# li-kunyi/CUT3R-SLAM

Hardware: AMD Instinct MI355X
Metric: frames/sec (ViT pointmap + covisibility-graph tracking step) on 640x480 (higher is better)
Workload: dtype f16

## Files before the change

cut3r_slam_amd/_lib.py:

```python
from __future__ import annotations

import ctypes as C
import os

_HERE = os.path.dirname(os.path.abspath(__file__))
LIB_PATH = os.path.join(_HERE, "libcut3r_hip.so")

c_void_p, c_int, c_float, c_ll = C.c_void_p, C.c_int, C.c_float, C.c_longlong


class GemmDesc(C.Structure):
    _fields_ = [
        ("A", c_void_p), ("B", c_void_p), ("C", c_void_p), ("bias", c_void_p), ("res1", c_void_p), ("res2", c_void_p),
        ("M", c_int), ("N", c_int), ("K", c_int), ("lda", c_int), ("ldb", c_int), ("ldc", c_int), ("ldr1", c_int),
        ("ldr2", c_int),
        ("act", c_int), ("out_f16", c_int), ("res1_f16", c_int), ("res2_f16", c_int),
        ("batch", c_int),
        ("strideA", c_ll), ("strideB", c_ll), ("strideC", c_ll), ("strideBias", c_ll), ("strideR1", c_ll),
        ("strideR2", c_ll),
        ("conv_k", c_int), ("H", c_int), ("W", c_int), ("Cin", c_int), ("conv_stride", c_int), ("Ho", c_int),
        ("Wo", c_int), ("relu_in", c_int),
        ("shuf", c_int), ("shuf_cout", c_int), ("shuf_Hin", c_int), ("shuf_Win", c_int),
        ("tile", c_int), ("stages", c_int),
        ("rope_pos", c_void_p), ("rope_table", c_void_p), ("rope_cols", c_int), ("rope_pmin", c_int), ("rope_npos", c_int),
# ... 13 lines not shown
    "cut3r_rope2d_qk": [c_void_p, c_void_p, c_int, c_void_p, c_int, c_int, c_int, c_int, c_ll, c_ll, c_ll, c_ll, c_float, c_float,
                        c_void_p],
    "cut3r_rope2d_tab": [c_void_p, c_void_p, c_ll, c_ll, c_void_p, c_void_p, c_ll, c_ll, c_int, c_int, c_void_p, c_int, c_int, c_float,
                         c_float, c_void_p],
    "cut3r_layernorm": [c_void_p, c_int, c_void_p, c_void_p, c_float, c_int, c_int, c_void_p, c_int, c_void_p, c_int,
                        c_void_p, c_void_p, c_void_p],
    "cut3r_layernorm_dual": [c_void_p, c_int, c_void_p, c_void_p, c_void_p, c_int, c_void_p, c_void_p, c_void_p, c_int, c_float, c_int,
                             c_int, c_void_p],
    "cut3r_gemm_f16": [C.POINTER(GemmDesc), c_void_p],
    "cut3r_gemm_tile_for": [C.POINTER(GemmDesc)],
    "cut3r_gemm_f16_pair": [C.POINTER(GemmDesc), C.POINTER(GemmDesc), c_void_p],
    "cut3r_rope2d_table": [c_void_p, c_int, c_int, c_int, c_float, c_float, c_void_p],
    "cut3r_gemv_f16w": [c_void_p, c_int, c_void_p, c_int, c_void_p, c_void_p, c_int, c_int, c_int, c_int, c_int,
                        c_void_p, c_int, c_int, c_void_p],
    "cut3r_attention_variant": [c_int],
    "cut3r_attention_f16": [c_void_p, c_void_p, c_void_p, c_void_p, c_int, c_int, c_int, c_int, c_int,
                            c_ll, c_ll, c_ll, c_ll, c_ll, c_ll, c_ll, c_ll, c_float, c_void_p],
    "cut3r_im2col_patch": [c_void_p, c_int, c_int, c_int, c_int, c_int, c_int, c_void_p, c_void_p],
    "cut3r_cast_f32_f16": [c_void_p, c_int, c_void_p, c_int, c_int, c_int, c_void_p],
    "cut3r_colmean": [c_void_p, c_int, c_int, c_int, c_void_p, c_void_p],
    "cut3r_colmean_batched": [c_void_p, c_int, c_ll, c_int, c_int, c_int, c_void_p, c_ll, c_void_p],
    "cut3r_upsample2x_nhwc": [c_void_p, c_void_p, c_int, c_int, c_int, c_int, c_void_p],
    "cut3r_dpt_final": [c_void_p, c_int, c_int, c_void_p, c_void_p, c_int, c_void_p, c_void_p, c_void_p],
    "cut3r_postprocess_pts": [c_void_p, c_int, c_int, c_int, c_void_p, c_void_p, c_void_p],
    "cut3r_postprocess_pose": [c_void_p, c_int, c_void_p, c_void_p],
    "cut3r_patch_overlap": [c_void_p, c_void_p, c_int, c_int, c_float, c_void_p, c_void_p, c_void_p],
    "cut3r_patch_overlap_chain": [c_void_p, c_void_p, c_int, c_int, c_int, c_float, C.c_double, c_void_p, c_void_p, c_void_p, c_void_p,
                                  c_void_p, c_void_p],
    "cut3r_overlap_fwd": [c_void_p, c_int, C.POINTER(c_float), c_float, c_void_p, c_int, c_float, c_float, c_float, c_float,
                          c_int, c_int, c_int, c_void_p, c_void_p],
# ... 119 lines not shown
```

cut3r_slam_amd/csrc/attention.hip:

```cpp
#include <atomic>
#include <cstdlib>
#include <type_traits>
#include "common.h"
#include "../../include/cut3r_hip.h"

namespace {

typedef __fp16 fp16x4_t __attribute__((ext_vector_type(4)));

DEVINL void halves(float x, float& lo, float& hi) {
    const auto r = __builtin_amdgcn_permlane32_swap(__float_as_uint(x), __float_as_uint(x), false, false);
    lo = __uint_as_float(r[0]);
    hi = __uint_as_float(r[1]);
}

struct AttnArgs {
    const h16* q; const h16* k; const h16* v; h16* o;
    int Nq, Nk;
    long long q_sb, q_sn, k_sb, k_sn, v_sb, v_sn, o_sb, o_sn;
    float scale_log2;
};

template <int D, int NW>
__global__ __launch_bounds__(NW * 64, (D <= 64 && NW == 4) ? 3 : 1) void attn_kernel(const AttnArgs a) {
    constexpr int NTHR = NW * 64;
    constexpr int KT = 64;
    constexpr int DQ = D / 16;
    constexpr int DP = (D + 31) / 32;
    constexpr int KS_LD = D + 8;
    constexpr int VS_BYTES = (64 * DP) % 128 == 0 ? 64 * DP + 64 : 64 * DP;
    constexpr int V_LD = VS_BYTES / 2;
    constexpr int CHUNKS = KT * (D / 8);
    constexpr int NCH = (CHUNKS + NTHR - 1) / NTHR;
    __shared__ __attribute__((aligned(16))) h16 Ks[KT * KS_LD];
    __shared__ __attribute__((aligned(16))) h16 Vs[KT * V_LD];

// ... 2 lines not shown
    const int h = blockIdx.y, b = blockIdx.z;
    const int q0 = blockIdx.x * (32 * NW) + wave * 32;
    const h16* qp = a.q + (size_t)b * a.q_sb + (size_t)h * D;
    const h16* kp = a.k + (size_t)b * a.k_sb + (size_t)h * D;
    const h16* vp = a.v + (size_t)b * a.v_sb + (size_t)h * D;

    for (int i = tid; i < KT * V_LD; i += NTHR) Vs[i] = (h16)0;

    half8_t qf[DQ];
    {
        int qr = q0 + r;
        if (qr > a.Nq - 1) qr = a.Nq - 1;
        const h16* qrow = qp + (size_t)qr * a.q_sn;
#pragma unroll
        for (int s = 0; s < DQ; s++) qf[s] = *reinterpret_cast<const half8_t*>(qrow + 16 * s + 8 * hh);
    }

    f32x16 ot[DP];
#pragma unroll
    for (int d = 0; d < DP; d++)
#pragma unroll
        for (int i = 0; i < 16; i++) ot[d][i] = 0.f;
    float m_run = -INFINITY, l_run = 0.f;
    const bool active = q0 < a.Nq;
    const int extra = (a.Nk > KT && (a.Nk % KT) == 1) ? 1 : 0;
    if (extra) {
        float dot = 0.f;
#pragma unroll
        for (int s = 0; s < DQ; s++) {
            const half8_t k0 = *reinterpret_cast<const half8_t*>(kp + 16 * s + 8 * hh);
// ... 265 lines not shown
        }
        asm volatile("s_waitcnt vmcnt(0)" ::: "memory");
        return;
    }

    half8_t qf[QB][DQ];
    f32x16 ot[QB][DP];
    float m_run[QB], l_run[QB];
#pragma unroll
    for (int qb = 0; qb < QB; qb++) {
        int qr = q0 + qb * 32 + r;
        if (qr > a.Nq - 1) qr = a.Nq - 1;
        const h16* qrow = qp + (size_t)qr * a.q_sn;
#pragma unroll
        for (int s = 0; s < DQ; s++) qf[qb][s] = *reinterpret_cast<const half8_t*>(qrow + 16 * s + 8 * hh);
#pragma unroll
        for (int d = 0; d < DP; d++)
#pragma unroll
            for (int i = 0; i < 16; i++) ot[qb][d][i] = 0.f;
        m_run[qb] = -INFINITY;
        l_run[qb] = 0.f;
        if (extra) {
            float dot = 0.f;
#pragma unroll
            for (int s = 0; s < DQ; s++) {
                const half8_t k0 = *reinterpret_cast<const half8_t*>(kp + 16 * s + 8 * hh);
#pragma unroll
                for (int j = 0; j < 8; j++) dot = fmaf((float)qf[qb][s][j], (float)k0[j], dot);
            }
            { float d0, d1; halves(dot, d0, d1); dot = d0 + d1; }
// ... 250 lines not shown
            dim3 grid((unsigned)(((HB + 7) / 8) * 8 * nblk));
            hipLaunchKernelGGL((attn_pipe_kernel<D, 1, 4, 4>), grid, dim3(256), 0, s, a, nblk, HB, H);
            return cut3r_check_launch();
        }
    }
    if (blocks128 >= nw4_min || D >= 128) {
        dim3 grid((a.Nq + 127) / 128, H, B);
        hipLaunchKernelGGL((attn_kernel<D, 4>), grid, dim3(256), 0, s, a);
    } else {
        dim3 grid((a.Nq + 63) / 64, H, B);
        hipLaunchKernelGGL((attn_kernel<D, 2>), grid, dim3(128), 0, s, a);
    }
    return cut3r_check_launch();
}

}

extern "C" int cut3r_attention_variant(int v) {
    if (v < 0) return g_attn_variant.load(std::memory_order_relaxed);
    return g_attn_variant.exchange(v ? 1 : 0, std::memory_order_relaxed);
}

extern "C" int cut3r_attention_f16(const void* q, const void* k, const void* v, void* out, int B, int H, int Nq, int Nk, int D,
                                   long long q_sb, long long q_sn, long long k_sb, long long k_sn, long long v_sb, long long v_sn,
                                   long long o_sb, long long o_sn, float scale, void* stream) {
    if (!q || !k || !v || !out || B <= 0 || H <= 0 || Nq <= 0 || Nk <= 0) return CUT3R_ERR_ARG;
    if (((uintptr_t)q | (uintptr_t)k | (uintptr_t)v) & 15) return CUT3R_ERR_ARG;
    if ((uintptr_t)out & 7) return CUT3R_ERR_ARG;
    if ((q_sn | k_sn | v_sn | q_sb | k_sb | v_sb) & 7) return CUT3R_ERR_ARG;
    if ((o_sn | o_sb) & 3) return CUT3R_ERR_ARG;
    AttnArgs a;
    a.q = (const h16*)q; a.k = (const h16*)k; a.v = (const h16*)v; a.o = (h16*)out;
    a.Nq = Nq; a.Nk = Nk;
    a.q_sb = q_sb; a.q_sn = q_sn; a.k_sb = k_sb; a.k_sn = k_sn; a.v_sb = v_sb; a.v_sn = v_sn; a.o_sb = o_sb; a.o_sn = o_sn;
    a.scale_log2 = scale * 1.44269504088896340736f;
    hipStream_t s = (hipStream_t)stream;
    switch (D) {
        case 16: return launch_attn<16>(a, B, H, s);
        case 32: return launch_attn<32>(a, B, H, s);
        case 48: return launch_attn<48>(a, B, H, s);
        case 64: return launch_attn<64>(a, B, H, s);
        case 128: return launch_attn<128>(a, B, H, s);
        default: return CUT3R_ERR_ARG;
    }
}
```

cut3r_slam_amd/csrc/elementwise.hip:

```cpp
#include "common.h"
#include "../../include/cut3r_hip.h"

namespace {

template <typename T> struct alignas(4 * sizeof(T)) Vec4 { T v[4]; };

template <typename T>
__global__ __launch_bounds__(256) void rope2d_kernel(T* __restrict__ tok, T* __restrict__ tok2, const int64_t* __restrict__ pos,
                                                     int N, int H, int D, long long sB, long long sN, long long sH, long long sB2,
                                                     long long sN2, float base, float fwd) {
    __shared__ float cs[2][2][64];
    const int t = blockIdx.x;
    const int b = t / N, n = t - b * N;
    const int Q = D >> 2;
    if (threadIdx.x < 2 * Q) {
        const int X = threadIdx.x / Q, q = threadIdx.x - X * Q;
        const float inv = fwd / powf(base, (float)q / (float)Q);
        const float fr = (float)pos[(size_t)t * 2 + X] * inv;
        cs[X][0][q] = cosf(fr);
        cs[X][1][q] = sinf(fr);
    }
    __syncthreads();
    const int Q4 = Q >> 2;
    const int per_tensor = H * 2 * Q4;
// ... 265 lines not shown
        *reinterpret_cast<half8_t*>(out + m * Kp + k) = o;
    }
}

__global__ __launch_bounds__(256) void cast_kernel(const float* __restrict__ x, int ldx, h16* __restrict__ y, int ldy, int M, int C4) {
    const size_t total = (size_t)M * C4;
    for (size_t i = blockIdx.x * (size_t)blockDim.x + threadIdx.x; i < total; i += (size_t)gridDim.x * blockDim.x) {
        const int c = (int)(i % C4);
        const size_t m = i / C4;
        f32x4 v = *reinterpret_cast<const f32x4*>(x + m * ldx + c * 4);
        half4_t o = {(h16)v[0], (h16)v[1], (h16)v[2], (h16)v[3]};
        *reinterpret_cast<half4_t*>(y + m * ldy + c * 4) = o;
    }
}

__global__ __launch_bounds__(256) void colmean_kernel(const float* __restrict__ x, int ldx, int M, int C, float* __restrict__ y,
                                                      long long sx, long long sy) {
    __shared__ float part[16][64];
    x += (size_t)blockIdx.y * sx;
    y += (size_t)blockIdx.y * sy;
    const int col = threadIdx.x & 63, rg = threadIdx.x >> 6;
    const int c = blockIdx.x * 64 + col;
    float s0 = 0.f, s1 = 0.f, s2 = 0.f, s3 = 0.f;
    if (c < C) {
        int m = rg;
        for (; m + 12 < M; m += 16) {
            s0 += x[(size_t)m * ldx + c];
            s1 += x[(size_t)(m + 4) * ldx + c];
            s2 += x[(size_t)(m + 8) * ldx + c];
            s3 += x[(size_t)(m + 12) * ldx + c];
// ... 319 lines not shown
    if (!img || !out || B <= 0 || C <= 0 || P <= 0 || (P & 7) || H % P || W % P) return CUT3R_ERR_ARG;
    const size_t total = (size_t)B * (H / P) * (W / P) * (C * P * P / 8);
    if (u8)
        hipLaunchKernelGGL((im2col_kernel<true>), dim3(grid_for(total)), dim3(256), 0, (hipStream_t)stream, img, B, C, H, W, P, (h16*)out);
    else
        hipLaunchKernelGGL((im2col_kernel<false>), dim3(grid_for(total)), dim3(256), 0, (hipStream_t)stream, img, B, C, H, W, P, (h16*)out);
    return cut3r_check_launch();
}

extern "C" int cut3r_cast_f32_f16(const float* x, int ldx, void* y, int ldy, int M, int C, void* stream) {
    if (!x || !y || M <= 0 || C <= 0 || (C & 3) || (ldx & 3) || (ldy & 3)) return CUT3R_ERR_ARG;
    hipLaunchKernelGGL(cast_kernel, dim3(grid_for((size_t)M * (C / 4))), dim3(256), 0, (hipStream_t)stream, x, ldx, (h16*)y, ldy, M, C / 4);
    return cut3r_check_launch();
}

extern "C" int cut3r_colmean(const float* x, int ldx, int M, int C, float* y, void* stream) {
    if (!x || !y || M <= 0 || C <= 0) return CUT3R_ERR_ARG;
    hipLaunchKernelGGL(colmean_kernel, dim3((C + 63) / 64), dim3(256), 0, (hipStream_t)stream, x, ldx, M, C, y, 0LL, 0LL);
    return cut3r_check_launch();
}

extern "C" int cut3r_colmean_batched(const float* x, int B, long long stride_x, int ldx, int M, int C, float* y, long long stride_y,
                                     void* stream) {
    if (!x || !y || B <= 0 || B > 65535 || M <= 0 || C <= 0) return CUT3R_ERR_ARG;
    hipLaunchKernelGGL(colmean_kernel, dim3((C + 63) / 64, B), dim3(256), 0, (hipStream_t)stream, x, ldx, M, C, y, stride_x, stride_y);
    return cut3r_check_launch();
}

extern "C" int cut3r_upsample2x_nhwc(const void* in, void* out, int B, int H, int W, int C, void* stream) {
    if (!in || !out || B <= 0 || H <= 0 || W <= 0 || C <= 0 || (C & 7)) return CUT3R_ERR_ARG;
// ... 51 lines not shown
```

cut3r_slam_amd/model.py:

```python
from __future__ import annotations

import gc

import math
import re
from dataclasses import dataclass
from typing import Dict, List, Optional

import torch

from . import ops
from .config import Cut3rConfig, production_config, state_dict_schema

F16, F32 = torch.float16, torch.float32


@dataclass
class ARCroco3DStereoOutput:
    ress: Optional[List[dict]] = None
    views: Optional[List[dict]] = None


class _Lin:

# ... 31 lines not shown
        self.dual_stream = _os.environ.get("CUT3R_DUAL_STREAM", "1") != "0"
        self.dual_ln = _os.environ.get("CUT3R_DUAL_LN", "1") != "0"
        self.pair_gemm = _os.environ.get("CUT3R_PAIR_GEMM", "0") != "0"
        self.pair_rows = int(_os.environ.get("CUT3R_PAIR_ROWS", "0"))
        self.fused_rope = int(_os.environ.get("CUT3R_FUSED_ROPE", "1"))
        self.rope48_rows = int(_os.environ.get("CUT3R_ROPE48_ROWS", "0"))
        self.head_overlap = _os.environ.get("CUT3R_HEAD_OVERLAP", "1") != "0"
        self.head_chunk = max(1, int(_os.environ.get("CUT3R_HEAD_CHUNK", "28")))
        self.ln_fold = int(_os.environ.get("CUT3R_LN_FOLD", "1"))
        self._head_stream = None
        self._side = None
        self._head_side = None
        self.kv_fork = _os.environ.get("CUT3R_KV_FORK", "0") != "0"
        self.kv_fork_rows = int(_os.environ.get("CUT3R_KV_FORK_ROWS", "2048"))
        self._kv_streams = None
        self._prep(state_dict)

    @classmethod
    def from_state_dict(cls, cfg, sd, device="cuda:0", **kw):
        return cls(cfg, sd, device, **kw)

    @classmethod
    def from_pretrained(cls, path: str, config: Optional[Cut3rConfig] = None, device="cuda:0", **kw):
        import argparse
        import os
        if not os.path.isfile(path):
            raise FileNotFoundError(f"{path}: no checkpoint (this runtime never fetches from a hub)")
        with torch.serialization.safe_globals([argparse.Namespace]):
            ckpt = torch.load(path, map_location="cpu", weights_only=True)
        sd = ckpt["model"] if "model" in ckpt else ckpt
# ... 24 lines not shown
            self.w[name] = _Lin(sd[key + ".weight"], sd.get(key + ".bias"), dev)

        def ln(name):
            self.w[name] = (f32(name + ".weight"), f32(name + ".bias"))

        def fold(name, w, b, norm):
            if not self.ln_fold or w.shape[1] % 64 or w.shape[0] % 4:
                return
            gam, bet = sd[norm + ".weight"].double(), sd[norm + ".bias"].double()
            wd = w.double()
            L = _Lin((wd * gam[None, :]).float(), None, dev)
            L.b = (wd @ bet + b.double()).to(device=dev, dtype=F32).contiguous()
            L.c = L.w.double().sum(1).to(F32).contiguous()
            self.w[name + "@ln"] = L

        def enc_block(p):
            ln(p + ".norm1"); lin(p + ".attn.qkv"); lin(p + ".attn.proj"); ln(p + ".norm2")
            lin(p + ".mlp.fc1"); lin(p + ".mlp.fc2")
            if self.ln_fold >= 2:
                fold(p + ".attn.qkv", sd[p + ".attn.qkv.weight"], sd[p + ".attn.qkv.bias"], p + ".norm1")
                fold(p + ".mlp.fc1", sd[p + ".mlp.fc1.weight"], sd[p + ".mlp.fc1.bias"], p + ".norm2")

        def dec_block(p, folded=True):
            ln(p + ".norm1"); lin(p + ".attn.qkv"); lin(p + ".attn.proj")
            ln(p + ".norm2"); ln(p + ".norm3"); ln(p + ".norm_y")
            lin(p + ".cross_attn.projq"); lin(p + ".cross_attn.proj")
            wkv = torch.cat([sd[p + ".cross_attn.projk.weight"], sd[p + ".cross_attn.projv.weight"]], 0)
            bkv = torch.cat([sd[p + ".cross_attn.projk.bias"], sd[p + ".cross_attn.projv.bias"]], 0)
            self.w[p + ".cross_attn.projkv"] = _Lin(wkv, bkv, dev)
            lin(p + ".mlp.fc1"); lin(p + ".mlp.fc2")
            if folded:
                fold(p + ".attn.qkv", sd[p + ".attn.qkv.weight"], sd[p + ".attn.qkv.bias"], p + ".norm1")
                fold(p + ".cross_attn.projq", sd[p + ".cross_attn.projq.weight"], sd[p + ".cross_attn.projq.bias"], p + ".norm2")
                fold(p + ".cross_attn.projkv", wkv, bkv, p + ".norm_y")
                fold(p + ".mlp.fc1", sd[p + ".mlp.fc1.weight"], sd[p + ".mlp.fc1.bias"], p + ".norm3")

        self.w["patch_embed"] = _Lin(sd["patch_embed.proj.weight"], sd["patch_embed.proj.bias"], dev)
        for i in range(cfg.enc_depth):
            enc_block(f"enc_blocks.{i}")
        ln("enc_norm")
        lin("decoder_embed"); lin("decoder_embed_state")
        for i in range(cfg.dec_depth):
            dec_block(f"dec_blocks.{i}"); dec_block(f"dec_blocks_state.{i}")
        ln("dec_norm"); ln("dec_norm_state")
        lin("pose_retriever.proj_q")
        for i in range(2):
            dec_block(f"pose_retriever.write_blocks.{i}", False); dec_block(f"pose_retriever.read_blocks.{i}", False)
# ... 86 lines not shown
        def prob(x, name, out, res, ex):
            ex = dict(ex or {})
            L = self.w[name + "@ln"] if ex.get("ln") is not None else self.w[name]
            if ex.get("ln") is not None:
                ex["ln"] = (ex["ln"], L.c, self.cfg.ln_eps)
            if ex.get("rope") is not None:
                r = ex["rope"]
                ex["rope"] = (r[0], r[1], self.cfg.rope_freq, r[2])
            return (x, L.w, out, L.b, res, {k: v for k, v in ex.items() if v is not None})
        ops.linear_pair(prob(x0, name0, out0, res0, ex0), prob(x1, name1, out1, res1, ex1), act)

    def _fuse_rope(self, pos, D, rows):
        dims = (64, 48) if (self.fused_rope == 2 or (self.fused_rope and rows <= self.rope48_rows)) else (64,)
        return self.fused_rope and pos is not None and D in dims and pos.is_contiguous() and pos.numel() == 2 * rows

    def _ln(self, x, name, out16=None, out32=None, mod=None):
        g, b = self.w[name]
        ops.layernorm(x, g, b, self.cfg.ln_eps, out16, out32, mod[0] if mod else None, mod[1] if mod else None)

    def _rope(self, t, pos):
        ops.rope_2d_pair(t, pos, None, None, self.cfg.rope_freq, 1.0)

    def _self_attn(self, tag, x_ln16, B, N, heads, pos, p, out, res, ln=None, emit=None):
        Cc = x_ln16.shape[1]
        D = Cc // heads
        sk = N == 1
        qkv = self.buf(tag + ".qkv", (B * N, 3 * Cc), F16)
        fuse = (not sk) and self._fuse_rope(pos, D, B * N)
        self._linear(x_ln16, p + ".qkv", qkv, skinny=sk, rope=(pos, 2 * Cc, D) if fuse else None, ln=ln)
        v5 = qkv.view(B, N, 3, heads, D)
        q, k, v = v5[:, :, 0], v5[:, :, 1], v5[:, :, 2]
        if pos is not None and not fuse:
            ops.rope_2d_pair(q, pos, k, pos, self.cfg.rope_freq, 1.0)
        a = self.buf(tag + ".attn", (B, N, heads, D), F16)
        ops.attention(q, k, v, a, D ** -0.5)
        self._linear(a.view(B * N, Cc), p + ".proj", out, res1=res, skinny=sk, emit=emit)

    def _mlp(self, tag, x_ln16, p, out, res, skinny=False, ln=None, emit=None):
        M = x_ln16.shape[0]
        hdim = self.w[p + ".fc1"].npad
        h = self.buf(tag + ".mlp_h", (M, hdim), F16)
        self._linear(x_ln16, p + ".fc1", h, act=1, skinny=skinny, ln=ln)
        self._linear(h, p + ".fc2", out, res1=res, skinny=skinny, emit=emit)

    def _encode(self, img: torch.Tensor):
        cfg = self.cfg
        B, _, H, W = img.shape
        P, E = cfg.patch_size, cfg.enc_embed_dim
        nh, nw = H // P, W // P
        N = nh * nw
# ... 98 lines not shown
                if not pre_ln:
                    self._ln(y, p + ".norm_y", out16=y16)
                self._linear(y16, p + ".cross_attn.projkv", kv, skinny=(Ny == 1), rope=(ypos, Cc, D) if fuse_k else None)
            if ypos is not None and not fuse_k:
                self._rope(k, ypos)

        if kv_only:
            kv_branch()
            return None
        if xs is not None:
            self._self_attn(tag, xs[0], B, Nx, heads, xpos, p + ".attn", out, x, ln=xs[1], emit=em)
        else:
            if not pre_ln:
                self._ln(x, p + ".norm1", out16=ln16)
            self._self_attn(tag, ln16, B, Nx, heads, xpos, p + ".attn", out, x, emit=em)
        q = self.buf(tag + ".q", (B, Nx, heads, D), F16)
        fuse_q = Nx > 1 and self._fuse_rope(xpos, D, B * Nx)
        if os_ is not None:
            self._linear(os_[0], p + ".cross_attn.projq", q.view(B * Nx, Cc), rope=(xpos, Cc, D) if fuse_q else None, ln=os_[1])
        else:
            self._ln(out, p + ".norm2", out16=ln16)
            self._linear(ln16, p + ".cross_attn.projq", q.view(B * Nx, Cc), skinny=(Nx == 1), rope=(xpos, Cc, D) if fuse_q else None)
        if xpos is not None and not fuse_q:
            self._rope(q, xpos)
        if kv_stream is not None:
            torch.cuda.current_stream().wait_stream(kv_stream)
        else:
            kv_branch()
        a = self.buf(tag + ".cattn", (B, Nx, heads, D), F16)
        ops.attention(q, k, v, a, D ** -0.5)
        self._linear(a.view(B * Nx, Cc), p + ".cross_attn.proj", out, res1=out, skinny=(Nx == 1), emit=em)
        if os_ is not None:
            self._mlp(tag, os_[0], p + ".mlp", out, out, ln=os_[1], emit=em)
        else:
            self._ln(out, p + ".norm3", out16=ln16)
            self._mlp(tag, ln16, p + ".mlp", out, out, skinny=(Nx == 1))
        return out

    def _dec_layer_pair(self, l, a, s_a, b, s_b, pos_img, pos_state, Wn, fork=False, xs=None, os_=None):
        cfg = self.cfg
        Cc = a.shape[1]
        ps, pi = f"dec_blocks_state.{l}", f"dec_blocks.{l}"
        Ni, Ns = a.shape[0] // Wn, s_a.shape[0] // Wn
        hs, hi = cfg.state_dec_num_heads, cfg.dec_num_heads
        Ds, Di = Cc // hs, Cc // hi
# ... 27 lines not shown
                    fn(S)
                fn(I)
                cur.wait_stream(self._side)
            else:
                fn(S)
                fn(I)

        if not fold_in:
            if self.dual_ln and Cc in (768, 1024, 1536):
                self._dual_norms(l, a, s_a)
            else:
                both(lambda sd: (self._ln(sd["x"], sd["p"] + ".norm1", out16=sd["ln16"]), self._ln(sd["y"], sd["p"] + ".norm_y", out16=sd["y16"])))
        for sd in (S, I):
            sd["fq"] = fr(sd["xpos"], sd["D"], Wn * sd["Nx"])
            sd["fk"] = fr(sd["ypos"], sd["D"], Wn * sd["Ny"])
        ex = lambda sd: {"rope": (sd["xpos"], 2 * Cc, sd["D"]) if sd["fq"] else None, "ln": sd["xst"] if fold_in else None}
        self._linear_pair(S["x16"] if fold_in else S["ln16"], ps + ".attn.qkv", S["qkv"], I["x16"] if fold_in else I["ln16"], pi + ".attn.qkv", I["qkv"],
                          ex0=ex(S), ex1=ex(I))

        def self_attn(sd):
            v5 = sd["qkv"].view(Wn, sd["Nx"], 3, sd["heads"], sd["D"])
            q, k, v = v5[:, :, 0], v5[:, :, 1], v5[:, :, 2]
            if sd["xpos"] is not None and not sd["fq"]:
                ops.rope_2d_pair(q, sd["xpos"], k, sd["xpos"], cfg.rope_freq, 1.0)
            ops.attention(q, k, v, sd["att"], sd["D"] ** -0.5)
        both(self_attn)
        self._linear_pair(S["att"].view(Wn * Ns, Cc), ps + ".attn.proj", S["out"], I["att"].view(Wn * Ni, Cc), pi + ".attn.proj", I["out"],
                          res0=S["x"], res1=I["x"], ex0=em(S), ex1=em(I))
        if not fold_out:
            both(lambda sd: self._ln(sd["out"], sd["p"] + ".norm2", out16=sd["ln16"]))
        ex = lambda sd: {"rope": (sd["xpos"], Cc, sd["D"]) if sd["fq"] else None, "ln": sd["ost"] if fold_out else None}
        self._linear_pair(S["o16"] if fold_out else S["ln16"], ps + ".cross_attn.projq", S["q"].view(Wn * Ns, Cc),
                          I["o16"] if fold_out else I["ln16"], pi + ".cross_attn.projq", I["q"].view(Wn * Ni, Cc), ex0=ex(S), ex1=ex(I))
        exk = lambda sd, other: {"rope": (sd["ypos"], Cc, sd["D"]) if sd["fk"] else None, "ln": other["xst"] if fold_in else None}
        self._linear_pair(I["x16"] if fold_in else S["y16"], ps + ".cross_attn.projkv", S["kv"], S["x16"] if fold_in else I["y16"], pi + ".cross_attn.projkv", I["kv"],
                          ex0=exk(S, I), ex1=exk(I, S))

        def cross_attn(sd):
            kv4 = sd["kv"].view(Wn, sd["Ny"], 2, sd["heads"], sd["D"])
            k, v = kv4[:, :, 0], kv4[:, :, 1]
            if not sd["fq"] or not sd["fk"]:
                qq = sd["q"] if not sd["fq"] else None
                kk = k if not sd["fk"] else None
                if qq is not None and kk is not None:
                    ops.rope_2d_pair(qq, sd["xpos"], kk, sd["ypos"], cfg.rope_freq, 1.0)
                elif qq is not None:
                    self._rope(qq, sd["xpos"])
                elif kk is not None:
                    self._rope(kk, sd["ypos"])
            ops.attention(sd["q"], k, v, sd["catt"], sd["D"] ** -0.5)
        both(cross_attn)
        self._linear_pair(S["catt"].view(Wn * Ns, Cc), ps + ".cross_attn.proj", S["out"], I["catt"].view(Wn * Ni, Cc), pi + ".cross_attn.proj", I["out"],
                          res0=S["out"], res1=I["out"], ex0=em(S), ex1=em(I))
        if not fold_out:
            both(lambda sd: self._ln(sd["out"], sd["p"] + ".norm3", out16=sd["ln16"]))
        ex = lambda sd: {"ln": sd["ost"] if fold_out else None}
        self._linear_pair(S["o16"] if fold_out else S["ln16"], ps + ".mlp.fc1", S["h"], I["o16"] if fold_out else I["ln16"], pi + ".mlp.fc1", I["h"], act=1,
                          ex0=ex(S), ex1=ex(I))
        self._linear_pair(S["h"], ps + ".mlp.fc2", S["out"], I["h"], pi + ".mlp.fc2", I["out"], res0=S["out"], res1=I["out"], ex0=em(S), ex1=em(I))

    def _dual_norms(self, l, a, s_a):
        pi, ps = f"dec_blocks.{l}", f"dec_blocks_state.{l}"
        Ci = a.shape[1]
        ops.layernorm_dual(a, *self.w[pi + ".norm1"], self.buf("deci.ln16", (a.shape[0], Ci), F16),
                           *self.w[ps + ".norm_y"], self.buf("decs.y16", (a.shape[0], Ci), F16), self.cfg.ln_eps)
# ... 421 lines not shown
```

cut3r_slam_amd/ops.py:

```python
from __future__ import annotations

import ctypes as C
import os
from typing import Optional

import torch

from . import _lib
from ._lib import GemmDesc, check

F16, F32 = torch.float16, torch.float32


def _stream():
    return C.c_void_p(torch.cuda.current_stream().cuda_stream)


def _p(t: Optional[torch.Tensor]):
    return C.c_void_p(t.data_ptr()) if t is not None else C.c_void_p(0)


def _req(cond, msg):
    if not cond:
        raise ValueError(msg)
# ... 312 lines not shown
    _cuda(X, W, out, bias, res)
    _req(X.dtype == F32 and W.dtype == F16 and out.dtype == F32, "dtypes: X fp32, W fp16, out fp32")
    M, K = X.shape
    N = W.shape[0]
    _req(W.shape[1] == K and out.shape == (M, N) and X.stride(1) == 1 and W.stride(1) == 1 and out.stride(1) == 1, "shapes")
    if bias is not None:
        _req(bias.dtype == F32 and bias.numel() == N, "bias")
    if res is not None:
        _req(res.dtype == F32 and res.shape == (M, N) and res.stride(1) == 1, "res")
    lib = _lib.load()
    check(lib.cut3r_gemv_f16w(_p(X), X.stride(0), _p(W), W.stride(0), _p(bias), _p(out), out.stride(0), M, N, K, act,
                              _p(res), res.stride(0) if res is not None else 0, int(silu_in), _stream()), "cut3r_gemv_f16w")
    return out


def attention(q, k, v, out, scale):
    _cuda(q, k, v, out)
    B, Nq, H, D = q.shape
    Nk = k.shape[1]
    for t in (q, k, v, out):
        _req(t.dtype == F16 and t.dim() == 4 and t.stride(3) == 1 and t.stride(2) == D, "attention operands: fp16 (B,N,H,D) views")
    _req(k.shape == (B, Nk, H, D) and v.shape == (B, Nk, H, D) and out.shape == (B, Nq, H, D), "attention shapes")
    _req(D in (16, 32, 48, 64, 128), f"unsupported head dim {D}")
    lib = _lib.load()
    check(lib.cut3r_attention_f16(_p(q), _p(k), _p(v), _p(out), B, H, Nq, Nk, D, q.stride(0), q.stride(1), k.stride(0),
                                  k.stride(1), v.stride(0), v.stride(1), out.stride(0), out.stride(1), float(scale),
                                  _stream()), f"cut3r_attention_f16 B={B} H={H} Nq={Nq} Nk={Nk} D={D}")
    return out


def im2col_patch(img, P, out):
    _cuda(img, out)
    _req(img.dim() == 4 and img.is_contiguous() and img.dtype in (F32, torch.uint8), "img [B,C,H,W] fp32|u8 contiguous")
    B, Cc, H, W = img.shape
    _req(out.dtype == F16 and out.is_contiguous() and out.shape == (B * (H // P) * (W // P), Cc * P * P), "im2col out shape")
    lib = _lib.load()
    check(lib.cut3r_im2col_patch(_p(img), int(img.dtype == torch.uint8), B, Cc, H, W, P, _p(out), _stream()), "cut3r_im2col_patch")
    return out


def cast_f16(x, out):
    _cuda(x, out)
    _req(x.dtype == F32 and out.dtype == F16 and x.shape == out.shape and x.dim() == 2, "cast: 2-D fp32 -> fp16")
    _req(x.stride(1) == 1 and out.stride(1) == 1, "unit inner stride")
    lib = _lib.load()
    check(lib.cut3r_cast_f32_f16(_p(x), x.stride(0), _p(out), out.stride(0), x.shape[0], x.shape[1], _stream()), "cut3r_cast_f32_f16")
    return out


def colmean(x, out):
    _cuda(x, out)
    _req(x.dtype == F32 and x.dim() == 2 and x.stride(1) == 1 and out.dtype == F32 and out.numel() == x.shape[1], "colmean")
    lib = _lib.load()
    check(lib.cut3r_colmean(_p(x), x.stride(0), x.shape[0], x.shape[1], _p(out), _stream()), "cut3r_colmean")
    return out


def colmean_batched(x, out):
    _cuda(x, out)
    _req(x.dtype == F32 and x.dim() == 3 and x.stride(2) == 1 and out.dtype == F32 and out.shape == (x.shape[0], x.shape[2]) and out.stride(1) == 1,
         "colmean_batched")
# ... 506 lines not shown
```

include/cut3r_hip.h:

```cpp
#ifndef CUT3R_HIP_H
#define CUT3R_HIP_H
#include <stdint.h>
#ifdef __cplusplus
extern "C" {
#endif

int cut3r_abi_version(void);

int cut3r_rope2d(void* tokens, int dtype, const int64_t* positions, int B, int N, int H, int D,
                 long long sB, long long sN, long long sH, float base, float fwd, void* stream);
int cut3r_rope2d_qk(void* q, void* k, int dtype, const int64_t* positions, int B, int N, int H, int D, long long q_sB,
                    long long q_sN, long long k_sB, long long k_sN, float base, float fwd, void* stream);

int cut3r_rope2d_tab(void* t0, const int64_t* pos0, long long ntok0, long long stride0, void* t1, const int64_t* pos1, long long ntok1,
                     long long stride1, int H, int D, const float* table, int pmin, int npos, float base, float fwd, void* stream);

int cut3r_layernorm(const float* x, int ldx, const float* gamma, const float* beta, float eps, int M, int C,
                    void* y16, int ld16, float* y32, int ld32, const float* mod_scale, const float* mod_shift,
                    void* stream);
int cut3r_layernorm_dual(const float* x, int ldx, const float* g1, const float* b1, void* y1, int ld1, const float* g2,
                         const float* b2, void* y2, int ld2, float eps, int M, int C, void* stream);

typedef struct cut3r_gemm_desc {
    const void* A;
// ... 26 lines not shown
    void* out16;
    int ld16;
} cut3r_gemm_desc;
int cut3r_gemm_f16(const cut3r_gemm_desc* d, void* stream);
int cut3r_rope2d_table(float* table, int pmin, int npos, int Q, float base, float fwd, void* stream);
int cut3r_gemm_tile_for(const cut3r_gemm_desc* d);
int cut3r_gemm_f16_pair(const cut3r_gemm_desc* d0, const cut3r_gemm_desc* d1, void* stream);

int cut3r_gemv_f16w(const float* X, int ldx, const void* W, int ldw, const float* bias, float* Y, int ldy,
                    int M, int N, int K, int act, const float* res, int ldr, int silu_in, void* stream);

int cut3r_attention_f16(const void* q, const void* k, const void* v, void* out, int B, int H, int Nq, int Nk, int D,
                        long long q_sb, long long q_sn, long long k_sb, long long k_sn, long long v_sb, long long v_sn,
                        long long o_sb, long long o_sn, float scale, void* stream);

int cut3r_attention_variant(int v);

int cut3r_im2col_patch(const void* img, int u8, int B, int C, int H, int W, int P, void* out, void* stream);
int cut3r_cast_f32_f16(const float* x, int ldx, void* y, int ldy, int M, int C, void* stream);
int cut3r_colmean(const float* x, int ldx, int M, int C, float* y, void* stream);
int cut3r_colmean_batched(const float* x, int B, long long stride_x, int ldx, int M, int C, float* y, long long stride_y, void* stream);

int cut3r_upsample2x_nhwc(const void* in, void* out, int B, int H, int W, int C, void* stream);
int cut3r_dpt_final(const void* in, int P, int Cin, const float* w, const float* b, int mode, float* pts, float* conf,
                    void* stream);
int cut3r_postprocess_pts(const float* raw, int P, int nch, int pos_z, float* pts, float* conf, void* stream);
int cut3r_postprocess_pose(const float* raw, int B, float* out, void* stream);

int cut3r_patch_overlap(const float* feat0, const float* feat1, int N, int C, float thr, void* ws, int32_t* count,
                        void* stream);
int cut3r_patch_overlap_chain(const float* feat_last, const float* feats, int B, int N, int C, float thr_sim, double thr_ratio,
                              const int32_t* forced_host, void* ws, int32_t* state, int32_t* counts, int32_t* decisions,
                              void* stream);

// ... 179 lines not shown
```

Measured before the change: 5847.

## Fuse query RoPE into attention kernel and elide single-key attention

Applies RoPE to the query inside the attention kernel at load time, using a precomputed cos/sin table. To make this work, the QKV weights are permuted to a K-first order so the fused GEMM RoPE only covers K, which removes the separate Q rope pass and its memory traffic. Separately, when there is a single key or value token, softmax is trivially one, so attention collapses to a V projection followed by the output projection, with a row-broadcast add for the residual. This adds trig and table work per query row in the kernel, plus more complex dispatch logic.

```diff
diff --git a/cut3r_slam_amd/_lib.py b/cut3r_slam_amd/_lib.py
--- a/cut3r_slam_amd/_lib.py
+++ b/cut3r_slam_amd/_lib.py
@@ -51,6 +51,8 @@
     "cut3r_gemv_f16w": [c_void_p, c_int, c_void_p, c_int, c_void_p, c_void_p, c_int, c_int, c_int, c_int, c_int,
                         c_void_p, c_int, c_int, c_void_p],
     "cut3r_attention_variant": [c_int],
+    "cut3r_attention_q_rope": [c_void_p, c_void_p, c_int, c_int, c_float, c_float],
+    "cut3r_rowbcast_add_f32": [c_void_p, c_int, c_void_p, c_int, c_void_p, c_int, c_int, c_int, c_int, c_void_p],
     "cut3r_attention_f16": [c_void_p, c_void_p, c_void_p, c_void_p, c_int, c_int, c_int, c_int, c_int,
                             c_ll, c_ll, c_ll, c_ll, c_ll, c_ll, c_ll, c_ll, c_float, c_void_p],
     "cut3r_im2col_patch": [c_void_p, c_int, c_int, c_int, c_int, c_int, c_int, c_void_p, c_void_p],
diff --git a/cut3r_slam_amd/csrc/attention.hip b/cut3r_slam_amd/csrc/attention.hip
--- a/cut3r_slam_amd/csrc/attention.hip
+++ b/cut3r_slam_amd/csrc/attention.hip
@@ -19,7 +19,76 @@
     int Nq, Nk;
     long long q_sb, q_sn, k_sb, k_sn, v_sb, v_sn, o_sb, o_sn;
     float scale_log2;
+    const int64_t* rp; const float* rtab;
+    int rpmin, rnpos;
+    float rbase, rfwd;
 };
+
+template <int D>
+DEVINL void rope_cs4(const AttnArgs& a, long long pp, int f0, float (&co)[4], float (&si)[4]) {
+    constexpr int Q = D / 4;
+    const long long pi = pp - a.rpmin;
+    if (pi >= 0 && pi < a.rnpos) {
+        const float* tc = a.rtab + pi * Q + f0;
+        const f32x4 c4 = *reinterpret_cast<const f32x4*>(tc), s4 = *reinterpret_cast<const f32x4*>(tc + (long long)a.rnpos * Q);
+#pragma unroll
+        for (int j = 0; j < 4; j++) { co[j] = c4[j]; si[j] = s4[j]; }
+    } else {
+#pragma unroll
+        for (int j = 0; j < 4; j++) {
+            const float inv = a.rfwd / powf(a.rbase, (float)(f0 + j) / (float)Q);
+            const float fr = (float)pp * inv;
+            co[j] = cosf(fr);
+            si[j] = sinf(fr);
+        }
+    }
+}
+
+template <int D, int DQ>
+DEVINL void rope_q(const AttnArgs& a, const h16* qrow, long long tok, int hh, half8_t (&qf)[DQ]) {
+    static_assert(D == 48 || D == 64, "query RoPE: head widths 48 and 64");
+    const long long py = a.rp[tok * 2], px = a.rp[tok * 2 + 1];
+    if constexpr (D == 64) {
+#pragma unroll
+        for (int X = 0; X < 2; X++) {
+            const half8_t u = qf[2 * X], v = qf[2 * X + 1];
+#pragma unroll
+            for (int g = 0; g < 2; g++) {
+                float co[4], si[4];
+                rope_cs4<D>(a, X ? px : py, 8 * hh + 4 * g, co, si);
+#pragma unroll
+                for (int e = 0; e < 4; e++) {
+                    const float uf = (float)u[4 * g + e], vf = (float)v[4 * g + e];
+                    float t1 = vf * si[e], t2 = uf * si[e];
+                    asm volatile("" : "+v"(t1), "+v"(t2));
+                    qf[2 * X][4 * g + e] = (h16)rope_rot(uf, co[e], -t1);
+                    qf[2 * X + 1][4 * g + e] = (h16)rope_rot(vf, co[e], t2);
+                }
+            }
+        }
+    } else {
+        constexpr int Q = D / 4;
+#pragma unroll
+        for (int s = 0; s < DQ; s++)
+#pragma unroll
+            for (int g = 0; g < 2; g++) {
+                const int c4 = 16 * s + 8 * hh + 4 * g;
+                const int X = c4 >= 2 * Q ? 1 : 0;
+                const int w = c4 - 2 * Q * X;
+                const bool is_u = w < Q;
+                const half4_t pt = *reinterpret_cast<const half4_t*>(qrow + (is_u ? c4 + Q : c4 - Q));
+                float co[4], si[4];
+                rope_cs4<D>(a, X ? px : py, is_u ? w : w - Q, co, si);
+#pragma unroll
+                for (int e = 0; e < 4; e++) {
+                    const float own = (float)qf[s][4 * g + e];
+                    float t = (float)pt[e] * si[e];
+                    asm volatile("" : "+v"(t));
+                    qf[s][4 * g + e] = (h16)rope_rot(own, co[e], is_u ? -t : t);
+                }
+            }
+    }
+}
 
 template <int D, int NW>
 __global__ __launch_bounds__(NW * 64, (D <= 64 && NW == 4) ? 3 : 1) void attn_kernel(const AttnArgs a) {
@@ -52,6 +121,9 @@
         const h16* qrow = qp + (size_t)qr * a.q_sn;
 #pragma unroll
         for (int s = 0; s < DQ; s++) qf[s] = *reinterpret_cast<const half8_t*>(qrow + 16 * s + 8 * hh);
+        if constexpr (D == 48 || D == 64) {
+            if (a.rp) rope_q<D, DQ>(a, qrow, (long long)b * a.Nq + qr, hh, qf);
+        }
     }
 
     f32x16 ot[DP];
@@ -347,6 +419,9 @@
         const h16* qrow = qp + (size_t)qr * a.q_sn;
 #pragma unroll
         for (int s = 0; s < DQ; s++) qf[qb][s] = *reinterpret_cast<const half8_t*>(qrow + 16 * s + 8 * hh);
+        if constexpr (D == 48 || D == 64) {
+            if (a.rp) rope_q<D, DQ>(a, qrow, (long long)b * a.Nq + qr, hh, qf[qb]);
+        }
 #pragma unroll
         for (int d = 0; d < DP; d++)
 #pragma unroll
@@ -627,6 +702,22 @@
     return cut3r_check_launch();
 }
 
+struct QRope {
+    const int64_t* pos = nullptr;
+    const float* table = nullptr;
+    int pmin = 0, npos = 0;
+    float base = 0.f, fwd = 0.f;
+};
+thread_local QRope t_qrope;
+
+}
+
+extern "C" int cut3r_attention_q_rope(const int64_t* positions, const float* table, int pmin, int npos, float base, float fwd) {
+    t_qrope = QRope{};
+    if (!positions) return CUT3R_OK;
+    if (!table || npos <= 0 || ((uintptr_t)table & 15) || ((uintptr_t)positions & 7)) return CUT3R_ERR_ARG;
+    t_qrope.pos = positions; t_qrope.table = table; t_qrope.pmin = pmin; t_qrope.npos = npos; t_qrope.base = base; t_qrope.fwd = fwd;
+    return CUT3R_OK;
 }
 
 extern "C" int cut3r_attention_variant(int v) {
@@ -637,6 +728,9 @@
 extern "C" int cut3r_attention_f16(const void* q, const void* k, const void* v, void* out, int B, int H, int Nq, int Nk, int D,
                                    long long q_sb, long long q_sn, long long k_sb, long long k_sn, long long v_sb, long long v_sn,
                                    long long o_sb, long long o_sn, float scale, void* stream) {
+    const QRope qr = t_qrope;
+    t_qrope = QRope{};
+    if (qr.pos && D != 48 && D != 64) return CUT3R_ERR_ARG;
     if (!q || !k || !v || !out || B <= 0 || H <= 0 || Nq <= 0 || Nk <= 0) return CUT3R_ERR_ARG;
     if (((uintptr_t)q | (uintptr_t)k | (uintptr_t)v) & 15) return CUT3R_ERR_ARG;
     if ((uintptr_t)out & 7) return CUT3R_ERR_ARG;
@@ -647,6 +741,7 @@
     a.Nq = Nq; a.Nk = Nk;
     a.q_sb = q_sb; a.q_sn = q_sn; a.k_sb = k_sb; a.k_sn = k_sn; a.v_sb = v_sb; a.v_sn = v_sn; a.o_sb = o_sb; a.o_sn = o_sn;
     a.scale_log2 = scale * 1.44269504088896340736f;
+    a.rp = qr.pos; a.rtab = qr.table; a.rpmin = qr.pmin; a.rnpos = qr.npos; a.rbase = qr.base; a.rfwd = qr.fwd;
     hipStream_t s = (hipStream_t)stream;
     switch (D) {
         case 16: return launch_attn<16>(a, B, H, s);
diff --git a/cut3r_slam_amd/csrc/elementwise.hip b/cut3r_slam_amd/csrc/elementwise.hip
--- a/cut3r_slam_amd/csrc/elementwise.hip
+++ b/cut3r_slam_amd/csrc/elementwise.hip
@@ -303,6 +303,19 @@
     }
 }
 
+__global__ __launch_bounds__(256) void rowbcast_add_kernel(const float* res, int ldr, const float* __restrict__ y, int ldy, float* out, int ldo,
+                                                           int B, int R, int C4) {
+    const size_t total = (size_t)B * R * C4;
+    for (size_t i = blockIdx.x * (size_t)blockDim.x + threadIdx.x; i < total; i += (size_t)gridDim.x * blockDim.x) {
+        const int c = (int)(i % C4);
+        const size_t m = i / C4;
+        const size_t b = m / R;
+        const f32x4 yv = *reinterpret_cast<const f32x4*>(y + b * ldy + c * 4);
+        const f32x4 rv = *reinterpret_cast<const f32x4*>(res + m * ldr + c * 4);
+        *reinterpret_cast<f32x4*>(out + m * ldo + c * 4) = yv + rv;
+    }
+}
+
 __global__ __launch_bounds__(256) void colmean_kernel(const float* __restrict__ x, int ldx, int M, int C, float* __restrict__ y,
                                                       long long sx, long long sy) {
     __shared__ float part[16][64];
@@ -652,6 +665,15 @@
     return cut3r_check_launch();
 }
 
+extern "C" int cut3r_rowbcast_add_f32(const float* res, int ldr, const float* y, int ldy, float* out, int ldo, int B, int R, int C,
+                                      void* stream) {
+    if (!res || !y || !out || B <= 0 || R <= 0 || C <= 0 || (C & 3) || (ldr & 3) || (ldy & 3) || (ldo & 3)) return CUT3R_ERR_ARG;
+    if (ldr < C || ldy < C || ldo < C || (((uintptr_t)res | (uintptr_t)y | (uintptr_t)out) & 15)) return CUT3R_ERR_ARG;
+    hipLaunchKernelGGL(rowbcast_add_kernel, dim3(grid_for((size_t)B * R * (C / 4))), dim3(256), 0, (hipStream_t)stream, res, ldr, y, ldy, out,
+                       ldo, B, R, C / 4);
+    return cut3r_check_launch();
+}
+
 extern "C" int cut3r_colmean(const float* x, int ldx, int M, int C, float* y, void* stream) {
     if (!x || !y || M <= 0 || C <= 0) return CUT3R_ERR_ARG;
     hipLaunchKernelGGL(colmean_kernel, dim3((C + 63) / 64), dim3(256), 0, (hipStream_t)stream, x, ldx, M, C, y, 0LL, 0LL);
diff --git a/cut3r_slam_amd/model.py b/cut3r_slam_amd/model.py
--- a/cut3r_slam_amd/model.py
+++ b/cut3r_slam_amd/model.py
@@ -69,6 +69,9 @@
         self.kv_fork = _os.environ.get("CUT3R_KV_FORK", "0") != "0"
         self.kv_fork_rows = int(_os.environ.get("CUT3R_KV_FORK_ROWS", "2048"))
         self._kv_streams = None
+        self.qrope = _os.environ.get("CUT3R_QROPE", "1") != "0"
+        self.onekey_elide = _os.environ.get("CUT3R_ONEKEY_ELIDE", "1") != "0"
+        self._kfirst = set()
         self._prep(state_dict)
 
     @classmethod
@@ -123,15 +126,28 @@
             L.c = L.w.double().sum(1).to(F32).contiguous()
             self.w[name + "@ln"] = L
 
+        def qkv_kfirst(name):
+            w, b = sd[name + ".weight"], sd.get(name + ".bias")
+            Cq = w.shape[0] // 3
+            perm = torch.cat([torch.arange(Cq, 2 * Cq), torch.arange(0, Cq), torch.arange(2 * Cq, 3 * Cq)])
+            w, b = w[perm], (b[perm] if b is not None else None)
+            self.w[name] = _Lin(w, b, dev)
+            self._kfirst.add(name)
+            return w, b
+
         def enc_block(p):
-            ln(p + ".norm1"); lin(p + ".attn.qkv"); lin(p + ".attn.proj"); ln(p + ".norm2")
+            ln(p + ".norm1"); wq, bq = qkv_kfirst(p + ".attn.qkv"); lin(p + ".attn.proj"); ln(p + ".norm2")
             lin(p + ".mlp.fc1"); lin(p + ".mlp.fc2")
             if self.ln_fold >= 2:
-                fold(p + ".attn.qkv", sd[p + ".attn.qkv.weight"], sd[p + ".attn.qkv.bias"], p + ".norm1")
+                fold(p + ".attn.qkv", wq, bq, p + ".norm1")
                 fold(p + ".mlp.fc1", sd[p + ".mlp.fc1.weight"], sd[p + ".mlp.fc1.bias"], p + ".norm2")
 
         def dec_block(p, folded=True):
-            ln(p + ".norm1"); lin(p + ".attn.qkv"); lin(p + ".attn.proj")
+            ln(p + ".norm1"); lin(p + ".attn.proj")
+            if folded:
+                wq, bq = qkv_kfirst(p + ".attn.qkv")
+            else:
+                lin(p + ".attn.qkv")
             ln(p + ".norm2"); ln(p + ".norm3"); ln(p + ".norm_y")
             lin(p + ".cross_attn.projq"); lin(p + ".cross_attn.proj")
             wkv = torch.cat([sd[p + ".cross_attn.projk.weight"], sd[p + ".cross_attn.projv.weight"]], 0)
@@ -139,7 +155,7 @@
             self.w[p + ".cross_attn.projkv"] = _Lin(wkv, bkv, dev)
             lin(p + ".mlp.fc1"); lin(p + ".mlp.fc2")
             if folded:
-                fold(p + ".attn.qkv", sd[p + ".attn.qkv.weight"], sd[p + ".attn.qkv.bias"], p + ".norm1")
+                fold(p + ".attn.qkv", wq, bq, p + ".norm1")
                 fold(p + ".cross_attn.projq", sd[p + ".cross_attn.projq.weight"], sd[p + ".cross_attn.projq.bias"], p + ".norm2")
                 fold(p + ".cross_attn.projkv", wkv, bkv, p + ".norm_y")
                 fold(p + ".mlp.fc1", sd[p + ".mlp.fc1.weight"], sd[p + ".mlp.fc1.bias"], p + ".norm3")
@@ -256,6 +272,9 @@
         dims = (64, 48) if (self.fused_rope == 2 or (self.fused_rope and rows <= self.rope48_rows)) else (64,)
         return self.fused_rope and pos is not None and D in dims and pos.is_contiguous() and pos.numel() == 2 * rows
 
+    def _q_rope(self, pos, D, B, N):
+        return bool(self.qrope and pos is not None and D in (48, 64) and pos.is_contiguous() and tuple(pos.shape) == (B, N, 2))
+
     def _ln(self, x, name, out16=None, out32=None, mod=None):
         g, b = self.w[name]
         ops.layernorm(x, g, b, self.cfg.ln_eps, out16, out32, mod[0] if mod else None, mod[1] if mod else None)
@@ -267,15 +286,26 @@
         Cc = x_ln16.shape[1]
         D = Cc // heads
         sk = N == 1
+        if sk and self.onekey_elide and ln is None:
+            L = self.w[p + ".qkv"]
+            v1 = self.buf(tag + ".v1", (B, Cc), F16)
+            ops.linear(x_ln16, L.w[2 * Cc:3 * Cc], v1, L.b[2 * Cc:3 * Cc] if L.b is not None else None, tile=16)
+            self._linear(v1, p + ".proj", out, res1=res, skinny=True, emit=emit)
+            return
         qkv = self.buf(tag + ".qkv", (B * N, 3 * Cc), F16)
+        kf = (p + ".qkv") in self._kfirst
         fuse = (not sk) and self._fuse_rope(pos, D, B * N)
-        self._linear(x_ln16, p + ".qkv", qkv, skinny=sk, rope=(pos, 2 * Cc, D) if fuse else None, ln=ln)
+        qr = self._q_rope(pos, D, B, N) and (kf or not fuse)
+        self._linear(x_ln16, p + ".qkv", qkv, skinny=sk, rope=(pos, Cc if qr else 2 * Cc, D) if fuse else None, ln=ln)
         v5 = qkv.view(B, N, 3, heads, D)
-        q, k, v = v5[:, :, 0], v5[:, :, 1], v5[:, :, 2]
+        q, k, v = v5[:, :, 1 if kf else 0], v5[:, :, 0 if kf else 1], v5[:, :, 2]
         if pos is not None and not fuse:
-            ops.rope_2d_pair(q, pos, k, pos, self.cfg.rope_freq, 1.0)
+            if qr:
+                ops.rope_2d_pair(k, pos, None, None, self.cfg.rope_freq, 1.0)
+            else:
+                ops.rope_2d_pair(q, pos, k, pos, self.cfg.rope_freq, 1.0)
         a = self.buf(tag + ".attn", (B, N, heads, D), F16)
-        ops.attention(q, k, v, a, D ** -0.5)
+        ops.attention(q, k, v, a, D ** -0.5, q_rope=(pos, self.cfg.rope_freq) if qr else None)
         self._linear(a.view(B * N, Cc), p + ".proj", out, res1=res, skinny=sk, emit=emit)
 
     def _mlp(self, tag, x_ln16, p, out, res, skinny=False, ln=None, emit=None):
@@ -404,21 +434,37 @@
             if not pre_ln:
                 self._ln(x, p + ".norm1", out16=ln16)
             self._self_attn(tag, ln16, B, Nx, heads, xpos, p + ".attn", out, x, emit=em)
+        if self.onekey_elide and Ny == 1 and em is None:
+            if kv_stream is not None:
+                torch.cuda.current_stream().wait_stream(kv_stream)
+            else:
+                kv_branch()
+            v1 = kv[:, Cc:]
+            if Nx == 1:
+                self._linear(v1, p + ".cross_attn.proj", out, res1=out, skinny=True)
+            else:
+                y1 = self.buf(tag + ".cproj1", (B, Cc), F32)
+                self._linear(v1, p + ".cross_attn.proj", y1)
+                ops.rowbcast_add(out, y1, out)
+            self._ln(out, p + ".norm3", out16=ln16)
+            self._mlp(tag, ln16, p + ".mlp", out, out, skinny=(Nx == 1))
+            return out
         q = self.buf(tag + ".q", (B, Nx, heads, D), F16)
-        fuse_q = Nx > 1 and self._fuse_rope(xpos, D, B * Nx)
+        qr = self._q_rope(xpos, D, B, Nx)
+        fuse_q = (not qr) and Nx > 1 and self._fuse_rope(xpos, D, B * Nx)
         if os_ is not None:
             self._linear(os_[0], p + ".cross_attn.projq", q.view(B * Nx, Cc), rope=(xpos, Cc, D) if fuse_q else None, ln=os_[1])
         else:
             self._ln(out, p + ".norm2", out16=ln16)
             self._linear(ln16, p + ".cross_attn.projq", q.view(B * Nx, Cc), skinny=(Nx == 1), rope=(xpos, Cc, D) if fuse_q else None)
-        if xpos is not None and not fuse_q:
+        if xpos is not None and not fuse_q and not qr:
             self._rope(q, xpos)
         if kv_stream is not None:
             torch.cuda.current_stream().wait_stream(kv_stream)
         else:
             kv_branch()
         a = self.buf(tag + ".cattn", (B, Nx, heads, D), F16)
-        ops.attention(q, k, v, a, D ** -0.5)
+        ops.attention(q, k, v, a, D ** -0.5, q_rope=(xpos, self.cfg.rope_freq) if qr else None)
         self._linear(a.view(B * Nx, Cc), p + ".cross_attn.proj", out, res1=out, skinny=(Nx == 1), emit=em)
         if os_ is not None:
             self._mlp(tag, os_[0], p + ".mlp", out, out, ln=os_[1], emit=em)
@@ -476,22 +522,28 @@
         for sd in (S, I):
             sd["fq"] = fr(sd["xpos"], sd["D"], Wn * sd["Nx"])
             sd["fk"] = fr(sd["ypos"], sd["D"], Wn * sd["Ny"])
-        ex = lambda sd: {"rope": (sd["xpos"], 2 * Cc, sd["D"]) if sd["fq"] else None, "ln": sd["xst"] if fold_in else None}
+            sd["kf"] = (sd["p"] + ".attn.qkv") in self._kfirst
+            sd["qr"] = self._q_rope(sd["xpos"], sd["D"], Wn, sd["Nx"]) and (sd["kf"] or not sd["fq"])
+            sd["qrope"] = (sd["xpos"], cfg.rope_freq) if sd["qr"] else None
+        ex = lambda sd: {"rope": (sd["xpos"], Cc if sd["qr"] else 2 * Cc, sd["D"]) if sd["fq"] else None, "ln": sd["xst"] if fold_in else None}
         self._linear_pair(S["x16"] if fold_in else S["ln16"], ps + ".attn.qkv", S["qkv"], I["x16"] if fold_in else I["ln16"], pi + ".attn.qkv", I["qkv"],
                           ex0=ex(S), ex1=ex(I))
 
         def self_attn(sd):
             v5 = sd["qkv"].view(Wn, sd["Nx"], 3, sd["heads"], sd["D"])
-            q, k, v = v5[:, :, 0], v5[:, :, 1], v5[:, :, 2]
+            q, k, v = v5[:, :, 1 if sd["kf"] else 0], v5[:, :, 0 if sd["kf"] else 1], v5[:, :, 2]
             if sd["xpos"] is not None and not sd["fq"]:
-                ops.rope_2d_pair(q, sd["xpos"], k, sd["xpos"], cfg.rope_freq, 1.0)
-            ops.attention(q, k, v, sd["att"], sd["D"] ** -0.5)
+                if sd["qr"]:
+                    ops.rope_2d_pair(k, sd["xpos"], None, None, cfg.rope_freq, 1.0)
+                else:
+                    ops.rope_2d_pair(q, sd["xpos"], k, sd["xpos"], cfg.rope_freq, 1.0)
+            ops.attention(q, k, v, sd["att"], sd["D"] ** -0.5, q_rope=sd["qrope"])
         both(self_attn)
         self._linear_pair(S["att"].view(Wn * Ns, Cc), ps + ".attn.proj", S["out"], I["att"].view(Wn * Ni, Cc), pi + ".attn.proj", I["out"],
                           res0=S["x"], res1=I["x"], ex0=em(S), ex1=em(I))
         if not fold_out:
             both(lambda sd: self._ln(sd["out"], sd["p"] + ".norm2", out16=sd["ln16"]))
-        ex = lambda sd: {"rope": (sd["xpos"], Cc, sd["D"]) if sd["fq"] else None, "ln": sd["ost"] if fold_out else None}
+        ex = lambda sd: {"rope": (sd["xpos"], Cc, sd["D"]) if (sd["fq"] and not sd["qr"]) else None, "ln": sd["ost"] if fold_out else None}
         self._linear_pair(S["o16"] if fold_out else S["ln16"], ps + ".cross_attn.projq", S["q"].view(Wn * Ns, Cc),
                           I["o16"] if fold_out else I["ln16"], pi + ".cross_attn.projq", I["q"].view(Wn * Ni, Cc), ex0=ex(S), ex1=ex(I))
         exk = lambda sd, other: {"rope": (sd["ypos"], Cc, sd["D"]) if sd["fk"] else None, "ln": other["xst"] if fold_in else None}
@@ -501,8 +553,8 @@
         def cross_attn(sd):
             kv4 = sd["kv"].view(Wn, sd["Ny"], 2, sd["heads"], sd["D"])
             k, v = kv4[:, :, 0], kv4[:, :, 1]
-            if not sd["fq"] or not sd["fk"]:
-                qq = sd["q"] if not sd["fq"] else None
+            if not (sd["fq"] or sd["qr"]) or not sd["fk"]:
+                qq = sd["q"] if not (sd["fq"] or sd["qr"]) else None
                 kk = k if not sd["fk"] else None
                 if qq is not None and kk is not None:
                     ops.rope_2d_pair(qq, sd["xpos"], kk, sd["ypos"], cfg.rope_freq, 1.0)
@@ -510,7 +562,7 @@
                     self._rope(qq, sd["xpos"])
                 elif kk is not None:
                     self._rope(kk, sd["ypos"])
-            ops.attention(sd["q"], k, v, sd["catt"], sd["D"] ** -0.5)
+            ops.attention(sd["q"], k, v, sd["catt"], sd["D"] ** -0.5, q_rope=sd["qrope"])
         both(cross_attn)
         self._linear_pair(S["catt"].view(Wn * Ns, Cc), ps + ".cross_attn.proj", S["out"], I["catt"].view(Wn * Ni, Cc), pi + ".cross_attn.proj", I["out"],
                           res0=S["out"], res1=I["out"], ex0=em(S), ex1=em(I))
diff --git a/cut3r_slam_amd/ops.py b/cut3r_slam_amd/ops.py
--- a/cut3r_slam_amd/ops.py
+++ b/cut3r_slam_amd/ops.py
@@ -350,7 +350,7 @@
     return out
 
 
-def attention(q, k, v, out, scale):
+def attention(q, k, v, out, scale, q_rope=None):
     _cuda(q, k, v, out)
     B, Nq, H, D = q.shape
     Nk = k.shape[1]
@@ -359,6 +359,13 @@
     _req(k.shape == (B, Nk, H, D) and v.shape == (B, Nk, H, D) and out.shape == (B, Nq, H, D), "attention shapes")
     _req(D in (16, 32, 48, 64, 128), f"unsupported head dim {D}")
     lib = _lib.load()
+    if q_rope is not None:
+        pos, base = q_rope[:2]
+        fwd = q_rope[2] if len(q_rope) > 2 else 1.0
+        _req(D in (48, 64), "query rope: head dims 48 and 64")
+        _req(pos.dtype == torch.int64 and pos.is_cuda and pos.is_contiguous() and pos.shape == (B, Nq, 2), "query rope positions int64 [B,Nq,2]")
+        tab = rope_table(q.device, base, fwd, D)
+        check(lib.cut3r_attention_q_rope(_p(pos), _p(tab), ROPE_PMIN, ROPE_NPOS, float(base), float(fwd)), "cut3r_attention_q_rope")
     check(lib.cut3r_attention_f16(_p(q), _p(k), _p(v), _p(out), B, H, Nq, Nk, D, q.stride(0), q.stride(1), k.stride(0),
                                   k.stride(1), v.stride(0), v.stride(1), out.stride(0), out.stride(1), float(scale),
                                   _stream()), f"cut3r_attention_f16 B={B} H={H} Nq={Nq} Nk={Nk} D={D}")
@@ -381,6 +388,18 @@
     _req(x.stride(1) == 1 and out.stride(1) == 1, "unit inner stride")
     lib = _lib.load()
     check(lib.cut3r_cast_f32_f16(_p(x), x.stride(0), _p(out), out.stride(0), x.shape[0], x.shape[1], _stream()), "cut3r_cast_f32_f16")
+    return out
+
+
+def rowbcast_add(res, y, out):
+    _cuda(res, y, out)
+    _req(res.dtype == F32 and y.dtype == F32 and out.dtype == F32 and res.dim() == 2 and y.dim() == 2 and out.shape == res.shape, "rowbcast_add: fp32 2-D")
+    B, Cc = y.shape
+    _req(B > 0 and res.shape[1] == Cc and res.shape[0] % B == 0 and Cc % 4 == 0, "rowbcast_add: res [B*R, C], y [B, C], C % 4 == 0")
+    _req(res.stride(1) == 1 and y.stride(1) == 1 and out.stride(1) == 1, "unit inner stride")
+    lib = _lib.load()
+    check(lib.cut3r_rowbcast_add_f32(_p(res), res.stride(0), _p(y), y.stride(0), _p(out), out.stride(0), B, res.shape[0] // B, Cc, _stream()),
+          "cut3r_rowbcast_add_f32")
     return out
 
 
diff --git a/include/cut3r_hip.h b/include/cut3r_hip.h
--- a/include/cut3r_hip.h
+++ b/include/cut3r_hip.h
@@ -64,10 +64,13 @@
                         long long q_sb, long long q_sn, long long k_sb, long long k_sn, long long v_sb, long long v_sn,
                         long long o_sb, long long o_sn, float scale, void* stream);
 
+int cut3r_attention_q_rope(const int64_t* positions, const float* table, int pmin, int npos, float base, float fwd);
+
 int cut3r_attention_variant(int v);
 
 int cut3r_im2col_patch(const void* img, int u8, int B, int C, int H, int W, int P, void* out, void* stream);
 int cut3r_cast_f32_f16(const float* x, int ldx, void* y, int ldy, int M, int C, void* stream);
+int cut3r_rowbcast_add_f32(const float* res, int ldr, const float* y, int ldy, float* out, int ldo, int B, int R, int C, void* stream);
 int cut3r_colmean(const float* x, int ldx, int M, int C, float* y, void* stream);
 int cut3r_colmean_batched(const float* x, int B, long long stride_x, int ldx, int M, int C, float* y, long long stride_y, void* stream);
 
```

After: 5704. -2.5%, worse.
